# abdelhakim96/Dynamic-Obstacle-Avoidance-MPC

Hardware: AMD Instinct MI355X
Metric: MPC solves/sec (N=20, 3 obstacles) (higher is better)
Workload: dtype f64; 1 GPU; C2: 1024 identical scenarios per GPU, N=20, Tf=2s, 3 moving obstacles; global_batch=1024, per_gpu_batch=1024, N=20, n_obst=3, parallelism=single GPU

## Files before the change

dynamic-obstacle-avoidance-mpc_amd/csrc/rti_kernel.hpp:

```cpp
#pragma once
#include <hip/hip_runtime.h>
#include <stdint.h>
#include <type_traits>

#ifdef MPC_PHASE_TIMING
#define MPC_T0() long long t_prev_ = clock64()
#define MPC_TICK(k) do { const long long t_now_ = clock64(); tacc_[k] += t_now_ - t_prev_; t_prev_ = t_now_; } while (0)
#else
#define MPC_T0() do {} while (0)
#define MPC_TICK(k) do {} while (0)
#endif

namespace mpc {

struct World {
    double xmin, xmax, ymin, ymax;
    int bug_compat_predict;
};

enum : int {
    kFuseShift = 1,
    kFusePlant = 2,
    kFuseObstacles = 4,
    kFuseResetOnFail = 8,
// ... 73 lines not shown
    const double *row = ref_row(p.yref, p.ref_off, p.ref_T, inst, i);
#pragma unroll
    for (int c = 0; c < 4; c++) r[c] = row[c];
    r[4] = has_u ? row[4] : 0.0; r[5] = has_u ? row[5] : 0.0;
}

template <bool IPAR>
__device__ __forceinline__ void load_ref_or_goal(const double *yref, const int32_t *off, int T, int inst, int i, bool has_u, const double gl[2], double r[6])
{
    if (IPAR && !yref) {
        r[0] = gl[0]; r[1] = gl[1]; r[2] = r[3] = r[4] = r[5] = 0.0;
        return;
    }
    const double *row = ref_row(yref, off, T, inst, i);
#pragma unroll
    for (int c = 0; c < 4; c++) r[c] = row[c];
    r[4] = has_u ? row[4] : 0.0; r[5] = has_u ? row[5] : 0.0;
}

__device__ __forceinline__ double ls_cost_ref(const double Wg[6], const double Weg[4], const double xi[5], const double ui[2], const double r[6], bool has_u)
{
    const double ex = xi[0] - r[0], ey = xi[1] - r[1], ev = xi[3] - r[2], eo = xi[4] - r[3];
    if (has_u) {
        const double ea = ui[0] - r[4], eal = ui[1] - r[5];
        return 0.5 * (Wg[0] * ex * ex + Wg[1] * ey * ey + Wg[2] * ev * ev + Wg[3] * eo * eo + Wg[4] * ea * ea + Wg[5] * eal * eal);
    }
    return 0.5 * (Weg[0] * ex * ex + Weg[1] * ey * ey + Weg[2] * ev * ev + Weg[3] * eo * eo);
}

static constexpr double kTLMin = 1e-11;
static constexpr double kFracToBoundary = 0.999995;
static constexpr double kMuDiverged = 1e8;
static constexpr double kMuCapFailed = 1e4;
static constexpr int kMuCapSettled = 20;

__device__ static constexpr double kGLC[4] = {0.069431844202973712388, 0.330009478207571867599,
                                              0.669990521792428132401, 0.930568155797026287612};
__device__ static constexpr double kGLB[4] = {0.173927422568726928687, 0.326072577431273071313,
                                              0.326072577431273071313, 0.173927422568726928687};

template <bool JAC>
__device__ __forceinline__ void dyn_step(const double x[5], const double u[2], double dt, double xn[5], double ae[6], double be[4])
{
    const double psi = x[2], v = x[3], om = x[4], a = u[0], al = u[1];
    double sx = 0, sy = 0, xpsi = 0, xv = 0, xom = 0, xa = 0, xal = 0, ypsi = 0, yv = 0, yom = 0, ya = 0, yal = 0;
#pragma unroll
    for (int j = 0; j < 4; j++) {
        const double tau = kGLC[j] * dt, w = kGLB[j] * dt;
        const double vj = v + a * tau;
        const double pj = psi + om * tau + 0.5 * al * tau * tau;
        double sj, cj;
        sincos(pj, &sj, &cj);
        const double wvc = w * vj * cj, wvs = w * vj * sj;
        sx += wvc; sy += wvs;
        if (JAC) {
            const double ht2 = 0.5 * tau * tau;
            xpsi -= wvs;        ypsi += wvc;
            xv += w * cj;       yv += w * sj;
            xom -= wvs * tau;   yom += wvc * tau;
            xa += w * tau * cj; ya += w * tau * sj;
            xal -= wvs * ht2;   yal += wvc * ht2;
        }
    }
    xn[0] = x[0] + sx; xn[1] = x[1] + sy;
    xn[2] = psi + om * dt + 0.5 * al * dt * dt;
    xn[3] = v + a * dt;
    xn[4] = om + al * dt;
    if (JAC) {
        ae[0] = xpsi; ae[1] = xv; ae[2] = xom; ae[3] = ypsi; ae[4] = yv; ae[5] = yom;
        be[0] = xa; be[1] = xal; be[2] = ya; be[3] = yal;
    }
}

__device__ __forceinline__ void coord_advance(double lo, double hi, double dt, double &x, double &v)
{
#pragma clang fp contract(off)
    const double av = fabs(v);
    const double n = v < 0 ? x - lo : hi - x;
    bool hit = false;
    double t_hit = 0.0;
    if (v != 0 && !(n > av * dt * (1.0 + 0x1p-50))) { t_hit = n / av; hit = t_hit <= dt; }
    if (hit) { const double a = v * t_hit, b = v * (dt - t_hit); x = x + (a - b); v = -v; }
    else { const double a = v * dt; x = x + a; }
}
__device__ __forceinline__ void obstacle_advance(const World w, double dt, double &x, double &vx, double &y, double &vy)
{
    coord_advance(w.xmin, w.xmax, dt, x, vx);
    coord_advance(w.ymin, w.ymax, dt, y, vy);
}
__device__ __forceinline__ void interp_guess(const double x0[5], double goal_y, int i, int N, double xg[5])
{
#pragma clang fp contract(off)
    const double dy = goal_y - x0[1];
    const double f = (double)i / (double)N;
    const double step = f * dy;
    xg[0] = x0[0] + f * (x0[0] - x0[0]);
    xg[1] = x0[1] + step;
    xg[2] = atan2(dy, 0.0);
    xg[3] = 0.0; xg[4] = 0.0;
}

__device__ __forceinline__ void obstacle_noise(double randomness, double vmax, double nx, double ny, double &vx, double &vy)
{
#pragma clang fp contract(off)
    const double rx = randomness * nx, ry = randomness * ny;
    const double fx = 1.0 + rx, fy = 1.0 + ry;
    vx = fmin(fmax(fx * vx, -vmax), vmax);
    vy = fmin(fmax(fy * vy, -vmax), vmax);
}

template <int CTRL>
__device__ __forceinline__ double dpp_f64(double v)
{
    const int lo = __builtin_amdgcn_mov_dpp(__double2loint(v), CTRL, 0xf, 0xf, true);
    const int hi = __builtin_amdgcn_mov_dpp(__double2hiint(v), CTRL, 0xf, 0xf, true);
    return __hiloint2double(hi, lo);
}
__device__ __forceinline__ double lane_value(double v, int src)
{
    const int lo = __builtin_amdgcn_readlane(__double2loint(v), src);
    const int hi = __builtin_amdgcn_readlane(__double2hiint(v), src);
    return __hiloint2double(hi, lo);
}
__device__ __forceinline__ int seg21_slot(int lane);
template <int G>
__device__ __forceinline__ double lane_value_seg(double v, int lane)
{
    if (G == 21) { const double a = lane_value(v, 0), b = lane_value(v, 21), c = lane_value(v, 42); return lane < 21 ? a : (lane < 42 ? b : c); }
    if (G == 64) return lane_value(v, 0);
    if (G == 32) { const double a = lane_value(v, 0), b = lane_value(v, 32); return lane < 32 ? a : b; }
    const double a = lane_value(v, 0), b = lane_value(v, 16), c = lane_value(v, 32), d = lane_value(v, 48);
    return lane < 16 ? a : (lane < 32 ? b : (lane < 48 ? c : d));
}
template <bool SUM> __device__ __forceinline__ double seg21_reduce(double v, int lane);
template <int G>
__device__ __forceinline__ double seg_max(double v, int lane)
{
    if (G == 21) return seg21_reduce<false>(v, lane);
    v = fmax(v, dpp_f64<0xB1>(v));
    v = fmax(v, dpp_f64<0x4E>(v));
    v = fmax(v, dpp_f64<0x141>(v));
    v = fmax(v, dpp_f64<0x140>(v));
    if (G == 16) return v;
    const double a = fmax(lane_value(v, 0), lane_value(v, 16)), b = fmax(lane_value(v, 32), lane_value(v, 48));
    if (G == 32) return lane < 32 ? a : b;
    return fmax(a, b);
}
template <int G>
__device__ __forceinline__ double seg_sum(double v, int lane)
{
    if (G == 21) return seg21_reduce<true>(v, lane);
    v += dpp_f64<0xB1>(v);
    v += dpp_f64<0x4E>(v);
    v += dpp_f64<0x141>(v);
    v += dpp_f64<0x140>(v);
    if (G == 16) return v;
    const double a = lane_value(v, 0) + lane_value(v, 16), b = lane_value(v, 32) + lane_value(v, 48);
    if (G == 32) return lane < 32 ? a : b;
    return a + b;
}

template <int G, bool SUM_A>
__device__ __forceinline__ void seg_reduce2(double &a, double &b, int lane)
{
    if (G == 21) { a = seg21_reduce<SUM_A>(a, lane); b = seg21_reduce<false>(b, lane); return; }
#define MPC_RED2_STEP(CTRL) { const double a2 = dpp_f64<CTRL>(a), b2 = dpp_f64<CTRL>(b); a = SUM_A ? a + a2 : fmax(a, a2); b = fmax(b, b2); }
// ... 2831 lines not shown
```

dynamic-obstacle-avoidance-mpc_amd/csrc/rti_split_kernel.hpp:

```cpp
#pragma once
#include "rti_kernel.hpp"
#include <type_traits>

namespace mpc {

template <int LPS, int NOBST, bool W2 = false, bool BLK2 = false>
struct SplitLds {
    using LT = typename std::conditional<W2, RowLdsC, RowLds>::type;
    static constexpr int NBL = 6 / LPS;
    static constexpr int NSL = (NOBST + LPS - 1) / LPS;
    static __host__ __device__ constexpr int results(int N) { return W2 ? 0 : (N + 1) * RowLds::HS; }
    static __host__ __device__ constexpr int total(int N, bool lookahead)
    {
        if (BLK2) return Blk2Lds::total(N) + (lookahead ? (N + 1) * NOBST * 2 : 0);
        return LT::total(N, 1) + results(N) + ((lookahead && !W2) ? (N + 1) * NOBST * 2 : 0);
    }
};

template <int K>
__device__ __forceinline__ double nth_of_six(double a0, double a1, double a2, double a3, double a4, double a5)
{
    if constexpr (K == 0) return a0; else if constexpr (K == 1) return a1; else if constexpr (K == 2) return a2;
    else if constexpr (K == 3) return a3; else if constexpr (K == 4) return a4; else return a5;
}

#ifdef MPC_FORCE_WAVES2
#define MPC_SPLIT_BOUNDS(W2) __launch_bounds__(64, 2)
#else
#define MPC_SPLIT_BOUNDS(W2) __launch_bounds__(64, (W2) ? 2 : 1)
#endif
template <int NOBST, int LPS, bool W2 = false, bool MASKED = false, bool BLK2 = false, bool REF = false, bool IPAR = false, bool OSEL = false>
__global__ MPC_SPLIT_BOUNDS(W2) void rti_split_kernel(const KParams p)
{
    static_assert(!OSEL || (IPAR && MASKED), "the obstacle masks are built on the per-instance parameters' code with a run-time row count");
    static_assert(!REF || !BLK2, "the per-stage reference is not built for the block-2 recursions");
    static_assert(!IPAR || REF, "the per-instance parameters are built on the per-stage reference's code");
    static_assert(LPS == 2 || LPS == 3, "two or three lanes per horizon stage");
    static_assert(!BLK2 || !W2, "the block-2 recursions exist on the dense layout only");
    using SL = SplitLds<LPS, NOBST, W2, BLK2>;
    using LT = typename SL::LT;
    constexpr int NBL = SL::NBL, NSL = SL::NSL;
    constexpr int kKK = 45;
    const int lane = threadIdx.x;
    const int inst = p.order ? p.order[blockIdx.x] : (int)blockIdx.x;
    const int N = p.N;
    const int nact = MASKED ? p.n_obst : NOBST;
    const int i = lane / LPS;
    const int h = lane - i * LPS;
    const bool own = (h == 0);
    uint32_t omask = 0u;
    if constexpr (OSEL) omask = omask_word(p.omask, __builtin_amdgcn_readfirstlane(inst), nact);
    const int osub = OSEL ? 31 - __builtin_clz(omask | 1u) : 0;
#define OBST_ON(j) (OSEL ? (((omask >> (j)) & 1u) != 0u) : ((j) < nact))
#define OBST_IN(j) (OSEL ? ((((omask >> (j)) & 1u) != 0u) ? (j) : osub) : ((j) < nact ? (j) : nact - 1))
    const bool act = (i <= N);
    const bool has_u = (i < N);
    const bool xb = (i >= 1) && (i < N || (i == N && p.bx_terminal));
    const double dt = p.dt, h2 = p.h2;
    int is_part1 = (h == 1), is_part2 = (h == 2);
    asm volatile("" : "+v"(is_part1), "+v"(is_part2));
    auto part_of = [&](auto sc, double a0, double a1, double a2, double a3, double a4, double a5) {
        constexpr int s = decltype(sc)::value;
        double r = nth_of_six<s>(a0, a1, a2, a3, a4, a5);
        r = is_part1 ? nth_of_six<NBL + s>(a0, a1, a2, a3, a4, a5) : r;
        if (LPS == 3) r = is_part2 ? nth_of_six<(2 * NBL + s) % 6>(a0, a1, a2, a3, a4, a5) : r;
        return r;
    };
    auto zpart_of = [&](auto sc, double v0, double v1, double v2, double v3, double v5, double v6) {
        return part_of(sc, v0, v1, v2, v3, v5, v6);
    };
    using slot0 = std::integral_constant<int, 0>; using slot1 = std::integral_constant<int, 1>; using slot2 = std::integral_constant<int, 2>;
    auto slots_of = [&](const double (&v)[7], double (&out)[NBL]) {
        out[0] = zpart_of(slot0{}, v[0], v[1], v[2], v[3], v[5], v[6]);
        out[1] = zpart_of(slot1{}, v[0], v[1], v[2], v[3], v[5], v[6]);
        if constexpr (NBL > 2) out[2] = zpart_of(slot2{}, v[0], v[1], v[2], v[3], v[5], v[6]);
    };

#ifdef MPC_PHASE_TIMING
    long long tacc_[16] = {0, 0, 0, 0, 0, 0, 0, 0, 0, 0, 0, 0, 0, 0, 0, 0};
#endif
    MPC_T0();
    double x0v[5], gl[2];
#pragma unroll
    for (int c = 0; c < 5; c++) x0v[c] = p.x0[(size_t)inst * 5 + c];
    gl[0] = p.goal[(size_t)inst * 2]; gl[1] = p.goal[(size_t)inst * 2 + 1];
    if constexpr (W2) {
#pragma unroll
        for (int c = 0; c < 5; c++) x0v[c] = wave_uniform(x0v[c]);
        gl[0] = wave_uniform(gl[0]); gl[1] = wave_uniform(gl[1]);
    }
    double *Xg = p.X + (size_t)inst * (N + 1) * 5, *Ug = p.U + (size_t)inst * N * 2;
    const int ep_word = ((p.fused & kFuseMetrics) && p.ep_flags) ? p.ep_flags[inst] : 0;
    double xi[5] = {0, 0, 0, 0, 0}, ui[2] = {0, 0}, xnext[5] = {0, 0, 0, 0, 0};
    if (act) {
#pragma unroll
        for (int c = 0; c < 5; c++) xi[c] = Xg[i * 5 + c];
    }
    if (has_u) {
        ui[0] = Ug[i * 2]; ui[1] = Ug[i * 2 + 1];
#pragma unroll
        for (int c = 0; c < 5; c++) xnext[c] = Xg[(i + 1) * 5 + c];
    }
    extern __shared__ double lds_raw[];
    const LT RL = [&]() {
        if constexpr (W2) return RowLdsC(lds_raw + RowLdsC::CT + RowLdsC::pad_front(N), N, lds_raw);
        else return RowLds(lds_raw + RowLds::pad_front(N), N, lds_raw + RowLds::total(N, 1));
    }();
    const Blk2Lds BL(lds_raw, N);
    const RowLds RV(lds_raw, N / 2, BL.R);
    const int Mb = N >> 1;
    const int mblk = i >> 1;
    const bool odd = (i & 1) != 0;
    double *lds_P = BLK2 ? lds_raw + Blk2Lds::total(N) : (W2 ? RL.H : lds_raw + LT::total(N, 1) + SL::results(N));
    auto of_part = [&](double v, int q) { return q == 0 ? v : (q == 1 ? from_right(v) : from_right(from_right(v))); };
    double pxy[NSL][2];
    if (p.obst) {
        if (lane < 2 * nact) {
            const int j = lane >> 1, c = lane & 1;
            const double *o = p.obst + ((size_t)inst * nact + j) * 4;
            double q = o[c], v = (c == 0 && !p.world.bug_compat_predict) ? o[2] : o[3];
            const double lo = c ? p.world.ymin : p.world.xmin, hi = c ? p.world.ymax : p.world.xmax;
            lds_P[lane] = q;
            for (int k = 1; k <= N; k++) {
                coord_advance(lo, hi, dt, q, v);
                lds_P[k * NOBST * 2 + lane] = q;
            }
        }
        wave_sync();
    }
    MPC_TICK(10);
    if (p.obst) {
#pragma unroll
        for (int s = 0; s < NSL; s++) {
            const int j = s * LPS + h, jj = OBST_IN(j);
            const double *src = lds_P + ((act ? i : 0) * NOBST + jj) * 2;
            pxy[s][0] = src[0]; pxy[s][1] = src[1];
        }
    } else {
#pragma unroll
        for (int s = 0; s < NSL; s++) {
            const int j = s * LPS + h, jj = OBST_IN(j);
            const double *src = p.P + (((size_t)inst * (N + 1) + (act ? i : 0)) * nact + jj) * 2;
            pxy[s][0] = src[0]; pxy[s][1] = src[1];
        }
    }
    if constexpr (OSEL) {
        if (omask == 0u) {
#pragma unroll
            for (int s = 0; s < NSL; s++) { pxy[s][0] = 0.0; pxy[s][1] = 0.0; }
        }
    }
    const bool ep_done = (ep_word & 1) != 0;
    double fin = gl[0] + gl[1] + ui[0] + ui[1];
#pragma unroll
    for (int c = 0; c < 5; c++) fin += x0v[c] + xi[c] + xnext[c];
#pragma unroll
    for (int s = 0; s < NSL; s++) fin += pxy[s][0] + pxy[s][1];

    MPC_TICK(11);
    double zpen = 0.0;
    {
        const double ex = x0v[0] - gl[0], ey = x0v[1] - gl[1];
        const double scale = p.slack_a * (ex * ex + ey * ey + x0v[3] * x0v[3] + x0v[4] * x0v[4] + p.slack_b);
        const double alpha_i = p.alpha ? p.alpha[(size_t)inst * (N + 1) + (act ? i : N)] : scale * (double)(N - i) / (double)N;
        zpen = alpha_i * (has_u ? p.ss : 1.0);
    }
    const bool vs = act && (i >= 1) && (p.soft_h ? (zpen > 0.0) : true);
    const bool soft = p.soft_h != 0;

    double lin0 = 0.0;
    double d0[5] = {0, 0, 0, 0, 0};
    StageLin S;
    S.a02 = S.a03 = S.a04 = S.a12 = S.a13 = S.a14 = S.b00 = S.b01 = S.b10 = S.b11 = 0.0; S.dt = dt; S.h2 = h2;
    double bb[5] = {0, 0, 0, 0, 0};
    if (has_u) {
        double xn[5], ae[6], be[4];
        dyn_step<true>(xi, ui, dt, xn, ae, be);
        S.a02 = ae[0]; S.a03 = ae[1]; S.a04 = ae[2]; S.a12 = ae[3]; S.a13 = ae[4]; S.a14 = ae[5];
        S.b00 = be[0]; S.b01 = be[1]; S.b10 = be[2]; S.b11 = be[3];
#pragma unroll
        for (int c = 0; c < 5; c++) { bb[c] = xn[c] - xnext[c]; lin0 = fmax(lin0, fabs(bb[c])); }
    }
    if (i == 0) {
#pragma unroll
        for (int c = 0; c < 5; c++) { d0[c] = x0v[c] - xi[c]; lin0 = fmax(lin0, fabs(d0[c])); }
    }
    StageLin Sa = S;
    double bba[5] = {0, 0, 0, 0, 0}, bh0[5] = {0, 0, 0, 0, 0};
    if constexpr (BLK2) {
        if (own && has_u) {
            double *w = BL.S + 16 * i;
            w[0] = bb[2]; w[1] = bb[3]; w[2] = S.a02; w[3] = S.a03; w[4] = S.a04; w[5] = bb[0]; w[6] = S.b00; w[7] = S.b01;
            w[8] = bb[4]; w[9] = 0.0; w[10] = S.a12; w[11] = S.a13; w[12] = S.a14; w[13] = bb[1]; w[14] = S.b10; w[15] = S.b11;
        }
        wave_sync();
        if (act && odd) {
            const double *w = BL.S + 16 * (i - 1);
            Sa.a02 = w[2]; Sa.a03 = w[3]; Sa.a04 = w[4]; Sa.b00 = w[6]; Sa.b01 = w[7];
            Sa.a12 = w[10]; Sa.a13 = w[11]; Sa.a14 = w[12]; Sa.b10 = w[14]; Sa.b11 = w[15];
            bba[0] = w[5]; bba[1] = w[13]; bba[2] = w[0]; bba[3] = w[1]; bba[4] = w[8];
        }
        if (own && odd && has_u) {
            const double Wh[5][10] = {
                {1.0, 0.0, Sa.a02 + S.a02, Sa.a03 + S.a03, fma(S.a02, dt, Sa.a04) + S.a04, 0.0,
                 fma(S.a03, dt, Sa.b00), fma(S.a04, dt, fma(S.a02, h2, Sa.b01)), S.b00, S.b01},
                {0.0, 1.0, Sa.a12 + S.a12, Sa.a13 + S.a13, fma(S.a12, dt, Sa.a14) + S.a14, 0.0,
                 fma(S.a13, dt, Sa.b10), fma(S.a14, dt, fma(S.a12, h2, Sa.b11)), S.b10, S.b11},
                {0.0, 0.0, 1.0, 0.0, 2.0 * dt, 0.0, 0.0, fma(dt, dt, h2), 0.0, h2},
                {0.0, 0.0, 0.0, 1.0, 0.0, 0.0, dt, 0.0, dt, 0.0},
                {0.0, 0.0, 0.0, 0.0, 1.0, 0.0, 0.0, dt, 0.0, dt}};
            double *w = BL.W + Blk2Lds::WS * mblk;
#pragma unroll
            for (int k = 0; k < 5; k++)
#pragma unroll
                for (int c = 0; c < 10; c++) w[k * 10 + c] = Wh[k][c];
            bh0[0] = fma(S.a04, bba[4], fma(S.a03, bba[3], fma(S.a02, bba[2], bba[0]))) + bb[0];
            bh0[1] = fma(S.a14, bba[4], fma(S.a13, bba[3], fma(S.a12, bba[2], bba[1]))) + bb[1];
            bh0[2] = fma(dt, bba[4], bba[2]) + bb[2]; bh0[3] = bba[3] + bb[3]; bh0[4] = bba[4] + bb[4];
        }
        if (own && act && (odd || i == N)) {
            double *hc = BL.H + Blk2Lds::HS * mblk;
#pragma unroll
            for (int e = 0; e < 100; e++) hc[e] = 0.0;
        }
    } else
    if constexpr (W2) {
        if (own && act) { double *hc = RL.H + LT::HS * i; hc[49] = 0.0; hc[50] = 0.0; }
        if (lane < 8) {
            const double c2[8] = {0.0, 0.0, 1.0, 0.0, dt, 0.0, 0.0, h2}, c3[8] = {0.0, 0.0, 0.0, 1.0, 0.0, 0.0, dt, 0.0}, c4[8] = {0.0, 0.0, 0.0, 0.0, 1.0, 0.0, 0.0, dt};
            double v2 = 0.0, v3 = 0.0, v4 = 0.0;
#pragma unroll
            for (int c = 0; c < 8; c++) if (lane == c) { v2 = c2[c]; v3 = c3[c]; v4 = c4[c]; }
// ... 678 lines not shown
            dz[0] = u0; dz[1] = u1;
        }
        }
#pragma unroll
        for (int c = 0; c < 7; c++) dz[c] += za[c];
        MPC_TICK(7);

        {
            double rmax = 0.0, rmaxd = 0.0;
            double dzs[NBL], dtl_[NBL], dth_[NBL], dll_[NBL], dlh_[NBL];
            slots_of(dz, dzs);
#pragma unroll
            for (int s = 0; s < NBL; s++) {
                dtl_[s] = dzs[s] + rdl[s]; dth_[s] = -dzs[s] + rdh[s];
                dll_[s] = -(ll[s] * tl[s] - smu + ppl[s] + ll[s] * dtl_[s]) * rtl[s];
                dlh_[s] = -(lh[s] * th[s] - smu + pph[s] + lh[s] * dth_[s]) * rth[s];
                if (bp[s]) {
                    rmax = fmax(rmax, fmax(-dtl_[s] * rtl[s], -dth_[s] * rth[s]));
                    rmaxd = fmax(rmaxd, fmax(-dll_[s] * rcp_nr(ll[s]), -dlh_[s] * rcp_nr(lh[s])));
                }
            }
            double dt1_[NSL], dl1_[NSL], dt2_[NSL], dl2_[NSL], ds_[NSL];
#pragma unroll
            for (int s = 0; s < NSL; s++) {
                const SoftT &o = so[s];
                const double y = ax[s] * dz[2] + ay[s] * dz[3];
                dt2_[s] = dl2_[s] = ds_[s] = 0.0;
                if (soft) {
                    const double db1 = (pp1[s] - smu) * rt1[s], db2 = (pp2[s] - smu) * rt2[s];
                    const double rsum = o.rs + (o.be1 + db1) + (o.be2 + db2);
                    ds_[s] = -(rsum + o.w1 * y) * o.rD;
                    dt1_[s] = o.rd1 + (y * (zpen + o.w2) - rsum) * o.rD;
                    dt2_[s] = o.rd2 + ds_[s];
                    dl2_[s] = -(l2[s] * t2[s] - smu + pp2[s] + l2[s] * dt2_[s]) * rt2[s];
                    if (sp[s]) { rmax = fmax(rmax, -dt2_[s] * rt2[s]); rmaxd = fmax(rmaxd, -dl2_[s] * rcp_nr(l2[s])); }
                } else dt1_[s] = o.rd1 + y;
                dl1_[s] = -(l1[s] * t1[s] - smu + pp1[s] + l1[s] * dt1_[s]) * rt1[s];
                if (sp[s]) { rmax = fmax(rmax, -dt1_[s] * rt1[s]); rmaxd = fmax(rmaxd, -dl1_[s] * rcp_nr(l1[s])); }
            }
            seg_reduce2<64, false>(rmax, rmaxd, lane);
            double alpha, alphad;
            ipm_step_lengths(rmax, rmaxd, alpha, alphad);
#ifndef MPC_PHASE_TIMING
            if (p.trace && lane == 0) p.trace[((size_t)inst * p.iter_max + it) * 4 + 2] = alpha;
#endif
            ipm_step_check(ipm, it, alpha, alphad, smu);
            ipm_polish_step<64>(p, ipm, lane, alpha, dz, stepl);
            if (running) {
#pragma unroll
                for (int c = 0; c < 7; c++) z[c] += alpha * dz[c];
#pragma unroll
                for (int s = 0; s < NBL; s++) {
                    zs[s] += alpha * dzs[s];
                    if (bp[s]) {
                        tl[s] = fmax(tl[s] + alpha * dtl_[s], p.tl_min); th[s] = fmax(th[s] + alpha * dth_[s], p.tl_min);
                        ll[s] = fmax(ll[s] + alphad * dll_[s], p.tl_min); lh[s] = fmax(lh[s] + alphad * dlh_[s], p.tl_min);
                        rtl[s] = rcp_nr(tl[s]); rth[s] = rcp_nr(th[s]);
                    }
                }
#pragma unroll
                for (int s = 0; s < NSL; s++) if (sp[s]) {
                    t1[s] = fmax(t1[s] + alpha * dt1_[s], p.tl_min); l1[s] = fmax(l1[s] + alphad * dl1_[s], p.tl_min);
                    rt1[s] = rcp_nr(t1[s]);
                    if (soft) {
                        sv[s] += alpha * ds_[s];
                        t2[s] = fmax(t2[s] + alpha * dt2_[s], p.tl_min); l2[s] = fmax(l2[s] + alphad * dl2_[s], p.tl_min);
                        rt2[s] = rcp_nr(t2[s]);
                    }
                }
                rhoPi = wave_uniform(rhoPi * (1.0 - alpha));
            }
        }
        MPC_TICK(8);
        if (!running) break;
    }

    if constexpr (!W2) {
        const double *xg = p.x0 + (size_t)inst * 5, *gg = p.goal + (size_t)inst * 2;
        asm volatile("" : "+v"(xg), "+v"(gg));
#pragma unroll
        for (int c = 0; c < 5; c++) x0v[c] = xg[c];
        gl[0] = gg[0]; gl[1] = gg[1];
    }
    const bool store = !ep_done;
    status = ipm_finite_step<64>(status, z, lane);
    if (status != 4) {
#pragma unroll
        for (int c = 0; c < 5; c++) xi[c] += z[2 + c];
        ui[0] += z[0]; ui[1] += z[1];
    }
    const double u_apply[2] = {lane_value(ui[0], 0), lane_value(ui[1], 0)};
    if ((p.fused & kFuseResetOnFail) && status == 4) {
        xi[0] = x0v[0]; xi[1] = x0v[1]; xi[2] = x0v[2]; xi[3] = 0.0; xi[4] = 0.0; ui[0] = ui[1] = 0.0;
        if (p.fused & kFuseInterpGuess) interp_guess(x0v, gl[1], i <= N ? i : N, N, xi);
    }
    if (store && own && (status != 4 || (p.fused & (kFuseResetOnFail | kFuseShift)))) {
        if (p.fused & kFuseShift) {
            if (act && i >= 1) {
#pragma unroll
                for (int c = 0; c < 5; c++) Xg[(i - 1) * 5 + c] = xi[c];
            }
            if (i == N) {
#pragma unroll
                for (int c = 0; c < 5; c++) Xg[N * 5 + c] = xi[c];
            }
            if (has_u && i >= 1) { Ug[(i - 1) * 2] = ui[0]; Ug[(i - 1) * 2 + 1] = ui[1]; }
            if (i == 0) { Ug[(N - 1) * 2] = 0.0; Ug[(N - 1) * 2 + 1] = 0.0; }
        } else {
            if (act) {
#pragma unroll
                for (int c = 0; c < 5; c++) Xg[i * 5 + c] = xi[c];
            }
            if (has_u) { Ug[i * 2] = ui[0]; Ug[i * 2 + 1] = ui[1]; }
        }
    }
    if (p.fused & (kFusePlant | kFuseObstacles | kFuseMetrics)) {
        double xp[5] = {x0v[0], x0v[1], x0v[2], x0v[3], x0v[4]};
        if ((p.fused & kFuseAliasBug) && (p.fused & kFuseResetOnFail) && status == 4) { xp[3] = 0.0; xp[4] = 0.0; }
        double xnew[5] = {xp[0], xp[1], xp[2], xp[3], xp[4]};
        if (p.fused & kFusePlant) dyn_step<false>(xp, u_apply, dt, xnew, nullptr, nullptr);
        if ((p.fused & kFusePlant) && lane == 0 && store && p.x0_rw) {
#pragma unroll
            for (int c = 0; c < 5; c++) p.x0_rw[(size_t)inst * 5 + c] = xnew[c];
        }
        double margin = INFINITY;
        if (p.obst && lane < nact) {
            const double *o = p.obst + ((size_t)inst * nact + lane) * 4;
            double ox = o[0], oy = o[1], ovx = o[2], ovy = o[3];
            if (p.fused & kFuseObstacles) {
                if (p.noise) obstacle_noise(p.randomness, p.vmax, p.noise[((size_t)inst * nact + lane) * 2], p.noise[((size_t)inst * nact + lane) * 2 + 1], ovx, ovy);
                obstacle_advance(p.world, dt, ox, ovx, oy, ovy);
                if (store && p.obst_rw) { double *w = p.obst_rw + ((size_t)inst * nact + lane) * 4; w[0] = ox; w[1] = oy; w[2] = ovx; w[3] = ovy; }
            }
            const double ddx = xnew[0] - ox, ddy = xnew[1] - oy;
            margin = sqrt(ddx * ddx + ddy * ddy) - (IPAR ? p.ip_rhit[(size_t)inst * nact + lane] : p.r_hit);
            if constexpr (OSEL) {
                if (!OBST_ON(lane) && !(p.fused & kFuseMarginAll)) margin = INFINITY;
            }
        }
        if (p.fused & kFuseMetrics) {
            margin = -seg_max<64>(-margin, lane);
            if (lane == 0 && store) {
                int fl = p.ep_flags[inst];
                if (xnew[0] < p.world.xmin || xnew[0] > p.world.xmax || xnew[1] < p.world.ymin || xnew[1] > p.world.ymax) fl |= 2;
                const double mm = fmin(p.ep_min_margin[inst], margin);
                p.ep_min_margin[inst] = mm;
                if (mm <= 0.0) fl |= 4;
                const double gx_ = xnew[0] - gl[0], gy_ = xnew[1] - gl[1];
                if (sqrt(gx_ * gx_ + gy_ * gy_) <= p.tol_goal) fl |= 1;
                else p.ep_steps[inst] += 1;
                p.ep_flags[inst] = fl;
            }
        }
    }
    if (lane == 0 && p.u0 && store) { p.u0[(size_t)inst * 2] = u_apply[0]; p.u0[(size_t)inst * 2 + 1] = u_apply[1]; }
    if (p.cost) {
        double J = 0.0;
        if (act) {
            if (IPAR && own) {
                double r[6];
                load_ref_or_goal<IPAR>(p.yref, p.ref_off, p.ref_T, inst, i, has_u, gl, r);
                const double wg[6] = {ipw[kIpWg], ipw[kIpWg + 1], ipw[kIpWg + 2], ipw[kIpWg + 3], ipw[kIpWg + 4], ipw[kIpWg + 5]};
                const double we[4] = {ipw[kIpWe], ipw[kIpWe + 1], ipw[kIpWe + 2], ipw[kIpWe + 3]};
                J = ls_cost_ref(wg, we, xi, ui, r, has_u);
            } else if (REF && own) {
                const double *row = ref_row(p.yref, p.ref_off, p.ref_T, inst, i);
                const double r[6] = {row[0], row[1], row[2], row[3], has_u ? row[4] : 0.0, has_u ? row[5] : 0.0};
                J = ls_cost_ref(p.Wg, p.Weg, xi, ui, r, has_u);
            } else if (own) {
                const double ex = xi[0] - gl[0], ey = xi[1] - gl[1];
                if (has_u) J = 0.5 * (p.Wg[0] * ex * ex + p.Wg[1] * ey * ey + p.Wg[2] * xi[3] * xi[3] + p.Wg[3] * xi[4] * xi[4]
                                      + p.Wg[4] * ui[0] * ui[0] + p.Wg[5] * ui[1] * ui[1]);
                else J = 0.5 * (p.Weg[0] * ex * ex + p.Weg[1] * ey * ey + p.Weg[2] * xi[3] * xi[3] + p.Weg[3] * xi[4] * xi[4]);
            }
#pragma unroll
            for (int s = 0; s < NSL; s++) if (OBST_ON(s * LPS + h)) {
                const double dx = xi[0] - pxy[s][0], dy = xi[1] - pxy[s][1];
                const double hv = dx * dx + dy * dy - ROW_R2(s);
                const double v = hv < 0 ? -hv : 0.0;
                J += zpen * (v + 0.5 * v * v);
            }
        }
        J = seg_sum<64>(J, lane);
        if (lane == 0 && store) p.cost[inst] = J;
    }
    if (lane == 0 && store) {
        if (p.iters_acc) p.iters_acc[inst] += it_done;
        if (p.status_acc) p.status_acc[inst] += (status == 4 ? 1 : 0) + (status == 2 ? 65536 : 0);
        if (p.status) p.status[inst] = status;
        if (p.iters) p.iters[inst] = it_done;
    }
    if constexpr (REF) {
        if ((p.fused & kFuseAdvanceRef) && lane == 0 && store && p.ref_off) p.ref_off[inst] += 1;
    }
#ifdef MPC_PHASE_TIMING
    __builtin_amdgcn_s_waitcnt(0);
    MPC_TICK(14);
    if (p.trace && lane == 0) { for (int k = 0; k < 16; k++) p.trace[((size_t)inst * p.iter_max) * 4 + k] = (double)tacc_[k]; }
#endif
}
#undef ROW_R2
#undef OBST_ON
#undef OBST_IN

}
```

Baseline: 7.179 million solves/s.

## Hoist epilogue global loads early and add wave-uniform fast path to obstacle prediction

Obstacle trajectory prediction now uses a walker that precomputes per-coordinate constants and takes a cheap add-only step when no lane in the wave is near a wall, falling back to the full bounce computation otherwise. The epilogue's global reads (obstacle states, noise, per-instance radii, metric accumulators, reference rows) are issued before the finite-check/store phase, so their latency overlaps that work instead of stalling on dependent reads later. Read-modify-write accumulators become plain stores of the preloaded value plus the increment. This costs extra registers held across the epilogue, which could affect occupancy. It also adds extra phase-timing ticks.

```diff
diff --git a/dynamic-obstacle-avoidance-mpc_amd/csrc/rti_kernel.hpp b/dynamic-obstacle-avoidance-mpc_amd/csrc/rti_kernel.hpp
--- a/dynamic-obstacle-avoidance-mpc_amd/csrc/rti_kernel.hpp
+++ b/dynamic-obstacle-avoidance-mpc_amd/csrc/rti_kernel.hpp
@@ -179,6 +179,28 @@
     if (v != 0 && !(n > av * dt * (1.0 + 0x1p-50))) { t_hit = n / av; hit = t_hit <= dt; }
     if (hit) { const double a = v * t_hit, b = v * (dt - t_hit); x = x + (a - b); v = -v; }
     else { const double a = v * dt; x = x + a; }
+}
+__device__ __forceinline__ void coord_walk(double lo, double hi, double dt, int N, double x, double v, double *dst, int stride)
+{
+#pragma clang fp contract(off)
+    double a, thr;
+    bool neg, still;
+    auto hoist = [&]() { const double av = fabs(v); a = v * dt; thr = av * dt * (1.0 + 0x1p-50); neg = v < 0; still = !(v != 0); };
+    auto step = [&]() {
+        const double n = neg ? x - lo : hi - x;
+        const bool near = !still && !(n > thr);
+        if (__builtin_amdgcn_ballot_w64(near) == 0) x = x + a;
+        else { coord_advance(lo, hi, dt, x, v); hoist(); }
+    };
+    hoist();
+    int k = 1;
+    for (; k < N; k += 2) {
+        step();
+        const double x1 = x;
+        step();
+        dst[k * stride] = x1; dst[(k + 1) * stride] = x;
+    }
+    if (k == N) { step(); dst[k * stride] = x; }
 }
 __device__ __forceinline__ void obstacle_advance(const World w, double dt, double &x, double &vx, double &y, double &vy)
 {
diff --git a/dynamic-obstacle-avoidance-mpc_amd/csrc/rti_split_kernel.hpp b/dynamic-obstacle-avoidance-mpc_amd/csrc/rti_split_kernel.hpp
--- a/dynamic-obstacle-avoidance-mpc_amd/csrc/rti_split_kernel.hpp
+++ b/dynamic-obstacle-avoidance-mpc_amd/csrc/rti_split_kernel.hpp
@@ -77,7 +77,7 @@
     };
 
 #ifdef MPC_PHASE_TIMING
-    long long tacc_[16] = {0, 0, 0, 0, 0, 0, 0, 0, 0, 0, 0, 0, 0, 0, 0, 0};
+    long long tacc_[24] = {0, 0, 0, 0, 0, 0, 0, 0, 0, 0, 0, 0, 0, 0, 0, 0, 0, 0, 0, 0, 0, 0, 0, 0};
 #endif
     MPC_T0();
     double x0v[5], gl[2];
@@ -114,17 +114,18 @@
     double *lds_P = BLK2 ? lds_raw + Blk2Lds::total(N) : (W2 ? RL.H : lds_raw + LT::total(N, 1) + SL::results(N));
     auto of_part = [&](double v, int q) { return q == 0 ? v : (q == 1 ? from_right(v) : from_right(from_right(v))); };
     double pxy[NSL][2];
+#ifdef MPC_PHASE_TIMING
+    __builtin_amdgcn_s_waitcnt(0);
+    MPC_TICK(16);
+#endif
     if (p.obst) {
         if (lane < 2 * nact) {
             const int j = lane >> 1, c = lane & 1;
             const double *o = p.obst + ((size_t)inst * nact + j) * 4;
-            double q = o[c], v = (c == 0 && !p.world.bug_compat_predict) ? o[2] : o[3];
+            const double q = o[c], v = (c == 0 && !p.world.bug_compat_predict) ? o[2] : o[3];
             const double lo = c ? p.world.ymin : p.world.xmin, hi = c ? p.world.ymax : p.world.xmax;
             lds_P[lane] = q;
-            for (int k = 1; k <= N; k++) {
-                coord_advance(lo, hi, dt, q, v);
-                lds_P[k * NOBST * 2 + lane] = q;
-            }
+            coord_walk(lo, hi, dt, N, q, v, lds_P + lane, NOBST * 2);
         }
         wave_sync();
     }
@@ -993,6 +994,43 @@
         gl[0] = gg[0]; gl[1] = gg[1];
     }
     const bool store = !ep_done;
+    const bool t_moves = (p.fused & (kFusePlant | kFuseObstacles | kFuseMetrics)) && p.obst && lane < nact;
+    double t_o[4] = {0, 0, 0, 0}, t_nz[2] = {0, 0}, t_rhit = p.r_hit;
+    if (t_moves) {
+        const size_t e = (size_t)inst * nact + lane;
+#pragma unroll
+        for (int c = 0; c < 4; c++) t_o[c] = p.obst[e * 4 + c];
+        if ((p.fused & kFuseObstacles) && p.noise) { t_nz[0] = p.noise[e * 2]; t_nz[1] = p.noise[e * 2 + 1]; }
+        if constexpr (IPAR) t_rhit = p.ip_rhit[e];
+    }
+    int t_fl = 0, t_steps = 0, t_iacc = 0, t_sacc = 0;
+    double t_mm = 0.0;
+    if (lane == 0 && store) {
+        if (p.fused & kFuseMetrics) {
+            t_fl = p.ep_flags[inst]; t_mm = p.ep_min_margin[inst];
+            if (p.ep_steps) t_steps = p.ep_steps[inst];
+        }
+        if (p.iters_acc) t_iacc = p.iters_acc[inst];
+        if (p.status_acc) t_sacc = p.status_acc[inst];
+    }
+    double t_r[6], t_r2[NSL];
+#pragma unroll
+    for (int s = 0; s < NSL; s++) t_r2[s] = p.r2;
+    if (p.cost && act) {
+        if constexpr (IPAR) { if (own) load_ref_or_goal<IPAR>(p.yref, p.ref_off, p.ref_T, inst, i, has_u, gl, t_r); }
+        else if constexpr (REF) {
+            if (own) {
+                const double *row = ref_row(p.yref, p.ref_off, p.ref_T, inst, i);
+#pragma unroll
+                for (int c = 0; c < 6; c++) t_r[c] = (c < 4 || has_u) ? row[c] : 0.0;
+            }
+        }
+        if constexpr (IPAR) {
+#pragma unroll
+            for (int s = 0; s < NSL; s++) if (OBST_ON(s * LPS + h)) t_r2[s] = ROW_R2(s);
+        }
+    }
+    MPC_TICK(17);
     status = ipm_finite_step<64>(status, z, lane);
     if (status != 4) {
 #pragma unroll
@@ -1024,6 +1062,7 @@
             if (has_u) { Ug[i * 2] = ui[0]; Ug[i * 2 + 1] = ui[1]; }
         }
     }
+    MPC_TICK(18);
     if (p.fused & (kFusePlant | kFuseObstacles | kFuseMetrics)) {
         double xp[5] = {x0v[0], x0v[1], x0v[2], x0v[3], x0v[4]};
         if ((p.fused & kFuseAliasBug) && (p.fused & kFuseResetOnFail) && status == 4) { xp[3] = 0.0; xp[4] = 0.0; }
@@ -1033,50 +1072,48 @@
 #pragma unroll
             for (int c = 0; c < 5; c++) p.x0_rw[(size_t)inst * 5 + c] = xnew[c];
         }
+        MPC_TICK(19);
         double margin = INFINITY;
-        if (p.obst && lane < nact) {
-            const double *o = p.obst + ((size_t)inst * nact + lane) * 4;
-            double ox = o[0], oy = o[1], ovx = o[2], ovy = o[3];
+        if (t_moves) {
+            double ox = t_o[0], oy = t_o[1], ovx = t_o[2], ovy = t_o[3];
             if (p.fused & kFuseObstacles) {
-                if (p.noise) obstacle_noise(p.randomness, p.vmax, p.noise[((size_t)inst * nact + lane) * 2], p.noise[((size_t)inst * nact + lane) * 2 + 1], ovx, ovy);
+                if (p.noise) obstacle_noise(p.randomness, p.vmax, t_nz[0], t_nz[1], ovx, ovy);
                 obstacle_advance(p.world, dt, ox, ovx, oy, ovy);
                 if (store && p.obst_rw) { double *w = p.obst_rw + ((size_t)inst * nact + lane) * 4; w[0] = ox; w[1] = oy; w[2] = ovx; w[3] = ovy; }
             }
             const double ddx = xnew[0] - ox, ddy = xnew[1] - oy;
-            margin = sqrt(ddx * ddx + ddy * ddy) - (IPAR ? p.ip_rhit[(size_t)inst * nact + lane] : p.r_hit);
+            margin = sqrt(ddx * ddx + ddy * ddy) - t_rhit;
             if constexpr (OSEL) {
                 if (!OBST_ON(lane) && !(p.fused & kFuseMarginAll)) margin = INFINITY;
             }
         }
+        MPC_TICK(20);
         if (p.fused & kFuseMetrics) {
             margin = -seg_max<64>(-margin, lane);
             if (lane == 0 && store) {
-                int fl = p.ep_flags[inst];
+                int fl = t_fl;
                 if (xnew[0] < p.world.xmin || xnew[0] > p.world.xmax || xnew[1] < p.world.ymin || xnew[1] > p.world.ymax) fl |= 2;
-                const double mm = fmin(p.ep_min_margin[inst], margin);
+                const double mm = fmin(t_mm, margin);
                 p.ep_min_margin[inst] = mm;
                 if (mm <= 0.0) fl |= 4;
                 const double gx_ = xnew[0] - gl[0], gy_ = xnew[1] - gl[1];
                 if (sqrt(gx_ * gx_ + gy_ * gy_) <= p.tol_goal) fl |= 1;
-                else p.ep_steps[inst] += 1;
+                else p.ep_steps[inst] = t_steps + 1;
                 p.ep_flags[inst] = fl;
             }
         }
     }
+    MPC_TICK(21);
     if (lane == 0 && p.u0 && store) { p.u0[(size_t)inst * 2] = u_apply[0]; p.u0[(size_t)inst * 2 + 1] = u_apply[1]; }
     if (p.cost) {
         double J = 0.0;
         if (act) {
             if (IPAR && own) {
-                double r[6];
-                load_ref_or_goal<IPAR>(p.yref, p.ref_off, p.ref_T, inst, i, has_u, gl, r);
                 const double wg[6] = {ipw[kIpWg], ipw[kIpWg + 1], ipw[kIpWg + 2], ipw[kIpWg + 3], ipw[kIpWg + 4], ipw[kIpWg + 5]};
                 const double we[4] = {ipw[kIpWe], ipw[kIpWe + 1], ipw[kIpWe + 2], ipw[kIpWe + 3]};
-                J = ls_cost_ref(wg, we, xi, ui, r, has_u);
+                J = ls_cost_ref(wg, we, xi, ui, t_r, has_u);
             } else if (REF && own) {
-                const double *row = ref_row(p.yref, p.ref_off, p.ref_T, inst, i);
-                const double r[6] = {row[0], row[1], row[2], row[3], has_u ? row[4] : 0.0, has_u ? row[5] : 0.0};
-                J = ls_cost_ref(p.Wg, p.Weg, xi, ui, r, has_u);
+                J = ls_cost_ref(p.Wg, p.Weg, xi, ui, t_r, has_u);
             } else if (own) {
                 const double ex = xi[0] - gl[0], ey = xi[1] - gl[1];
                 if (has_u) J = 0.5 * (p.Wg[0] * ex * ex + p.Wg[1] * ey * ey + p.Wg[2] * xi[3] * xi[3] + p.Wg[3] * xi[4] * xi[4]
@@ -1086,7 +1123,7 @@
 #pragma unroll
             for (int s = 0; s < NSL; s++) if (OBST_ON(s * LPS + h)) {
                 const double dx = xi[0] - pxy[s][0], dy = xi[1] - pxy[s][1];
-                const double hv = dx * dx + dy * dy - ROW_R2(s);
+                const double hv = dx * dx + dy * dy - t_r2[s];
                 const double v = hv < 0 ? -hv : 0.0;
                 J += zpen * (v + 0.5 * v * v);
             }
@@ -1094,9 +1131,10 @@
         J = seg_sum<64>(J, lane);
         if (lane == 0 && store) p.cost[inst] = J;
     }
+    MPC_TICK(22);
     if (lane == 0 && store) {
-        if (p.iters_acc) p.iters_acc[inst] += it_done;
-        if (p.status_acc) p.status_acc[inst] += (status == 4 ? 1 : 0) + (status == 2 ? 65536 : 0);
+        if (p.iters_acc) p.iters_acc[inst] = t_iacc + it_done;
+        if (p.status_acc) p.status_acc[inst] = t_sacc + (status == 4 ? 1 : 0) + (status == 2 ? 65536 : 0);
         if (p.status) p.status[inst] = status;
         if (p.iters) p.iters[inst] = it_done;
     }
@@ -1106,7 +1144,7 @@
 #ifdef MPC_PHASE_TIMING
     __builtin_amdgcn_s_waitcnt(0);
     MPC_TICK(14);
-    if (p.trace && lane == 0) { for (int k = 0; k < 16; k++) p.trace[((size_t)inst * p.iter_max) * 4 + k] = (double)tacc_[k]; }
+    if (p.trace && lane == 0) { for (int k = 0; k < 24 && k < 4 * p.iter_max; k++) p.trace[((size_t)inst * p.iter_max) * 4 + k] = (double)tacc_[k]; }
 #endif
 }
 #undef ROW_R2
```

Result: no change. 7.222 million solves/s (median of 6 runs) (+0.6%).

## Hoist obstacle step and epilogue loads early; batch clear-path obstacle prediction by four

Applied to the files above, without the earlier changes.

Obstacle prediction now advances four steps at a time when no wall bounce can occur in that window, and falls back to the exact per-step bounce logic otherwise. The kernel also loads obstacle state, noise and the per-instance accumulators near the start or before the final step. It advances the plant obstacles into LDS early, so the epilogue no longer waits on dependent global reads. The tail is restructured into a dedicated path that reorders the finite check, plant step, metrics, cost and stores. This adds code size and register pressure and duplicates epilogue logic that must stay in sync with the old path.

```diff
diff --git a/dynamic-obstacle-avoidance-mpc_amd/csrc/rti_kernel.hpp b/dynamic-obstacle-avoidance-mpc_amd/csrc/rti_kernel.hpp
--- a/dynamic-obstacle-avoidance-mpc_amd/csrc/rti_kernel.hpp
+++ b/dynamic-obstacle-avoidance-mpc_amd/csrc/rti_kernel.hpp
@@ -179,6 +179,22 @@
     if (v != 0 && !(n > av * dt * (1.0 + 0x1p-50))) { t_hit = n / av; hit = t_hit <= dt; }
     if (hit) { const double a = v * t_hit, b = v * (dt - t_hit); x = x + (a - b); v = -v; }
     else { const double a = v * dt; x = x + a; }
+}
+__device__ __forceinline__ bool coord_advance4_clear(double lo, double hi, double dt, double x, double v, double out[4])
+{
+#pragma clang fp contract(off)
+    const double av = fabs(v);
+    const double thr = av * dt * (1.0 + 0x1p-50), a = v * dt;
+    const bool neg = v < 0, still = !(v != 0);
+    bool clear = true;
+#pragma unroll
+    for (int j = 0; j < 4; j++) {
+        const double n = neg ? x - lo : hi - x;
+        clear = clear && (still || n > thr);
+        x = x + a;
+        out[j] = x;
+    }
+    return clear;
 }
 __device__ __forceinline__ void obstacle_advance(const World w, double dt, double &x, double &vx, double &y, double &vy)
 {
diff --git a/dynamic-obstacle-avoidance-mpc_amd/csrc/rti_split_kernel.hpp b/dynamic-obstacle-avoidance-mpc_amd/csrc/rti_split_kernel.hpp
--- a/dynamic-obstacle-avoidance-mpc_amd/csrc/rti_split_kernel.hpp
+++ b/dynamic-obstacle-avoidance-mpc_amd/csrc/rti_split_kernel.hpp
@@ -113,6 +113,17 @@
     const bool odd = (i & 1) != 0;
     double *lds_P = BLK2 ? lds_raw + Blk2Lds::total(N) : (W2 ? RL.H : lds_raw + LT::total(N, 1) + SL::results(N));
     auto of_part = [&](double v, int q) { return q == 0 ? v : (q == 1 ? from_right(v) : from_right(from_right(v))); };
+    constexpr bool FX = !W2 && !BLK2 && !(LPS == 2 && NOBST > 5);
+    const bool obst_step = p.obst && (p.fused & (kFusePlant | kFuseObstacles | kFuseMetrics)) && lane < nact;
+    double og[4] = {0, 0, 0, 0}, onz[2] = {0, 0};
+    if constexpr (FX) {
+        if (obst_step) {
+            const double *o = p.obst + ((size_t)inst * nact + lane) * 4;
+#pragma unroll
+            for (int c = 0; c < 4; c++) og[c] = o[c];
+            if ((p.fused & kFuseObstacles) && p.noise) { onz[0] = p.noise[((size_t)inst * nact + lane) * 2]; onz[1] = p.noise[((size_t)inst * nact + lane) * 2 + 1]; }
+        }
+    }
     double pxy[NSL][2];
     if (p.obst) {
         if (lane < 2 * nact) {
@@ -121,7 +132,20 @@
             double q = o[c], v = (c == 0 && !p.world.bug_compat_predict) ? o[2] : o[3];
             const double lo = c ? p.world.ymin : p.world.xmin, hi = c ? p.world.ymax : p.world.xmax;
             lds_P[lane] = q;
-            for (int k = 1; k <= N; k++) {
+            int k = 1;
+            if constexpr (FX) {
+                for (; k + 3 <= N; k += 4) {
+                    double q4[4];
+                    if (coord_advance4_clear(lo, hi, dt, q, v, q4)) q = q4[3];
+                    else {
+#pragma unroll
+                        for (int j = 0; j < 4; j++) { coord_advance(lo, hi, dt, q, v); q4[j] = q; }
+                    }
+#pragma unroll
+                    for (int j = 0; j < 4; j++) lds_P[(k + j) * NOBST * 2 + lane] = q4[j];
+                }
+            }
+            for (; k <= N; k++) {
                 coord_advance(lo, hi, dt, q, v);
                 lds_P[k * NOBST * 2 + lane] = q;
             }
@@ -148,6 +172,18 @@
         if (omask == 0u) {
 #pragma unroll
             for (int s = 0; s < NSL; s++) { pxy[s][0] = 0.0; pxy[s][1] = 0.0; }
+        }
+    }
+    if constexpr (FX) {
+        if (p.obst) wave_sync();
+        if (obst_step) {
+            if (p.fused & kFuseObstacles) {
+                if (p.noise) obstacle_noise(p.randomness, p.vmax, onz[0], onz[1], og[2], og[3]);
+                obstacle_advance(p.world, dt, og[0], og[2], og[1], og[3]);
+            }
+            double *w = lds_P + 4 * lane;
+#pragma unroll
+            for (int c = 0; c < 4; c++) w[c] = og[c];
         }
     }
     const bool ep_done = (ep_word & 1) != 0;
@@ -992,6 +1028,136 @@
         for (int c = 0; c < 5; c++) x0v[c] = xg[c];
         gl[0] = gg[0]; gl[1] = gg[1];
     }
+    if constexpr (FX) {
+        const bool store = !ep_done;
+        const bool lane0s = (lane == 0) && store;
+        double ox = 0.0, oy = 0.0, ovx = 0.0, ovy = 0.0;
+        if (obst_step) {
+            const double *w = lds_P + 4 * lane;
+            ox = w[0]; oy = w[1]; ovx = w[2]; ovy = w[3];
+        }
+        int acc_it = 0, acc_st = 0, ep_fl = 0, ep_inc = 0;
+        double ep_mm = 0.0;
+        if (lane0s) {
+            if (p.iters_acc) acc_it = p.iters_acc[inst];
+            if (p.status_acc) acc_st = p.status_acc[inst];
+            if (p.fused & kFuseMetrics) { ep_fl = p.ep_flags[inst]; ep_mm = p.ep_min_margin[inst]; }
+        }
+        status = ipm_finite_step<64>(status, z, lane);
+        if (status != 4) {
+#pragma unroll
+            for (int c = 0; c < 5; c++) xi[c] += z[2 + c];
+            ui[0] += z[0]; ui[1] += z[1];
+        }
+        const double u_apply[2] = {lane_value(ui[0], 0), lane_value(ui[1], 0)};
+        if ((p.fused & kFuseResetOnFail) && status == 4) {
+            xi[0] = x0v[0]; xi[1] = x0v[1]; xi[2] = x0v[2]; xi[3] = 0.0; xi[4] = 0.0; ui[0] = ui[1] = 0.0;
+            if (p.fused & kFuseInterpGuess) interp_guess(x0v, gl[1], i <= N ? i : N, N, xi);
+        }
+        const bool fused_step = (p.fused & (kFusePlant | kFuseObstacles | kFuseMetrics)) != 0;
+        double xnew[5] = {x0v[0], x0v[1], x0v[2], x0v[3], x0v[4]};
+        if (fused_step) {
+            double xp[5] = {x0v[0], x0v[1], x0v[2], x0v[3], x0v[4]};
+            if ((p.fused & kFuseAliasBug) && (p.fused & kFuseResetOnFail) && status == 4) { xp[3] = 0.0; xp[4] = 0.0; }
+#pragma unroll
+            for (int c = 0; c < 5; c++) xnew[c] = xp[c];
+            if (p.fused & kFusePlant) dyn_step<false>(xp, u_apply, dt, xnew, nullptr, nullptr);
+            double margin = INFINITY;
+            if (obst_step) {
+                const double ddx = xnew[0] - ox, ddy = xnew[1] - oy;
+                margin = sqrt(ddx * ddx + ddy * ddy) - (IPAR ? p.ip_rhit[(size_t)inst * nact + lane] : p.r_hit);
+                if constexpr (OSEL) {
+                    if (!OBST_ON(lane) && !(p.fused & kFuseMarginAll)) margin = INFINITY;
+                }
+            }
+            if (p.fused & kFuseMetrics) {
+                margin = -seg_max<64>(-margin, lane);
+                if (lane0s) {
+                    if (xnew[0] < p.world.xmin || xnew[0] > p.world.xmax || xnew[1] < p.world.ymin || xnew[1] > p.world.ymax) ep_fl |= 2;
+                    ep_mm = fmin(ep_mm, margin);
+                    if (ep_mm <= 0.0) ep_fl |= 4;
+                    const double gx_ = xnew[0] - gl[0], gy_ = xnew[1] - gl[1];
+                    if (sqrt(gx_ * gx_ + gy_ * gy_) <= p.tol_goal) ep_fl |= 1;
+                    else ep_inc = 1;
+                }
+            }
+        }
+        double J = 0.0;
+        if (p.cost) {
+            if (act) {
+                if (IPAR && own) {
+                    double r[6];
+                    load_ref_or_goal<IPAR>(p.yref, p.ref_off, p.ref_T, inst, i, has_u, gl, r);
+                    const double wg[6] = {ipw[kIpWg], ipw[kIpWg + 1], ipw[kIpWg + 2], ipw[kIpWg + 3], ipw[kIpWg + 4], ipw[kIpWg + 5]};
+                    const double we[4] = {ipw[kIpWe], ipw[kIpWe + 1], ipw[kIpWe + 2], ipw[kIpWe + 3]};
+                    J = ls_cost_ref(wg, we, xi, ui, r, has_u);
+                } else if (REF && own) {
+                    const double *row = ref_row(p.yref, p.ref_off, p.ref_T, inst, i);
+                    const double r[6] = {row[0], row[1], row[2], row[3], has_u ? row[4] : 0.0, has_u ? row[5] : 0.0};
+                    J = ls_cost_ref(p.Wg, p.Weg, xi, ui, r, has_u);
+                } else if (own) {
+                    const double ex = xi[0] - gl[0], ey = xi[1] - gl[1];
+                    if (has_u) J = 0.5 * (p.Wg[0] * ex * ex + p.Wg[1] * ey * ey + p.Wg[2] * xi[3] * xi[3] + p.Wg[3] * xi[4] * xi[4]
+                                          + p.Wg[4] * ui[0] * ui[0] + p.Wg[5] * ui[1] * ui[1]);
+                    else J = 0.5 * (p.Weg[0] * ex * ex + p.Weg[1] * ey * ey + p.Weg[2] * xi[3] * xi[3] + p.Weg[3] * xi[4] * xi[4]);
+                }
+#pragma unroll
+                for (int s = 0; s < NSL; s++) if (OBST_ON(s * LPS + h)) {
+                    const double dx = xi[0] - pxy[s][0], dy = xi[1] - pxy[s][1];
+                    const double hv = dx * dx + dy * dy - ROW_R2(s);
+                    const double v = hv < 0 ? -hv : 0.0;
+                    J += zpen * (v + 0.5 * v * v);
+                }
+            }
+            J = seg_sum<64>(J, lane);
+        }
+        if (store && own && (status != 4 || (p.fused & (kFuseResetOnFail | kFuseShift)))) {
+            if (p.fused & kFuseShift) {
+                if (act && i >= 1) {
+#pragma unroll
+                    for (int c = 0; c < 5; c++) Xg[(i - 1) * 5 + c] = xi[c];
+                }
+                if (i == N) {
+#pragma unroll
+                    for (int c = 0; c < 5; c++) Xg[N * 5 + c] = xi[c];
+                }
+                if (has_u && i >= 1) { Ug[(i - 1) * 2] = ui[0]; Ug[(i - 1) * 2 + 1] = ui[1]; }
+                if (i == 0) { Ug[(N - 1) * 2] = 0.0; Ug[(N - 1) * 2 + 1] = 0.0; }
+            } else {
+                if (act) {
+#pragma unroll
+                    for (int c = 0; c < 5; c++) Xg[i * 5 + c] = xi[c];
+                }
+                if (has_u) { Ug[i * 2] = ui[0]; Ug[i * 2 + 1] = ui[1]; }
+            }
+        }
+        if (fused_step) {
+            if ((p.fused & kFusePlant) && lane0s && p.x0_rw) {
+#pragma unroll
+                for (int c = 0; c < 5; c++) p.x0_rw[(size_t)inst * 5 + c] = xnew[c];
+            }
+            if (obst_step && (p.fused & kFuseObstacles) && store && p.obst_rw) {
+                double *w = p.obst_rw + ((size_t)inst * nact + lane) * 4;
+                w[0] = ox; w[1] = oy; w[2] = ovx; w[3] = ovy;
+            }
+            if ((p.fused & kFuseMetrics) && lane0s) {
+                p.ep_min_margin[inst] = ep_mm;
+                if (ep_inc) p.ep_steps[inst] += 1;
+                p.ep_flags[inst] = ep_fl;
+            }
+        }
+        if (lane0s) {
+            if (p.u0) { p.u0[(size_t)inst * 2] = u_apply[0]; p.u0[(size_t)inst * 2 + 1] = u_apply[1]; }
+            if (p.cost) p.cost[inst] = J;
+            if (p.iters_acc) p.iters_acc[inst] = acc_it + it_done;
+            if (p.status_acc) p.status_acc[inst] = acc_st + (status == 4 ? 1 : 0) + (status == 2 ? 65536 : 0);
+            if (p.status) p.status[inst] = status;
+            if (p.iters) p.iters[inst] = it_done;
+        }
+        if constexpr (REF) {
+            if ((p.fused & kFuseAdvanceRef) && lane0s && p.ref_off) p.ref_off[inst] += 1;
+        }
+    } else {
     const bool store = !ep_done;
     status = ipm_finite_step<64>(status, z, lane);
     if (status != 4) {
@@ -1103,6 +1269,7 @@
     if constexpr (REF) {
         if ((p.fused & kFuseAdvanceRef) && lane == 0 && store && p.ref_off) p.ref_off[inst] += 1;
     }
+    }
 #ifdef MPC_PHASE_TIMING
     __builtin_amdgcn_s_waitcnt(0);
     MPC_TICK(14);
```

Result: faster. 7.161 million solves/s before, 7.279 million solves/s after (median of 6 runs) (+1.7%).
